# IDEA-Research/MP-Former

Measured on AMD Instinct MI355X. Metric: training images/sec COCO-instance R50 1024x1024, higher is better.
Workload: dtype bf16 (backbone, decoder) + f32 (pixel decoder, losses), as the reference's AMP; 1 GPU; COCO-instance R50, 100 queries, 80 classes, 1024x1024: full train step = R50 backbone + MSDeformAttn pixel decoder (6 layers) + MP masked decoder (9 layers, NUM_DN 1) + Hungarian matching + 60 losses + backward + grad all-reduce + clip + AdamW; head_only_workload=False, global_batch=2, per_gpu_batch=2, parallelism=dp1, msda_offsets=init, full=False, autograd_threads=backward on the launch thread, miopen_find_db=shipped

## Files before the change

include/mpformer_hip.h:

```cpp
#ifndef MPFORMER_HIP_H
#define MPFORMER_HIP_H

#include <stddef.h>
#include <stdint.h>

#ifdef __cplusplus
extern "C" {
#endif

enum { MPF_F32 = 0, MPF_F64 = 1, MPF_BF16 = 2, MPF_U8 = 3, MPF_BITS = 4  };

enum {
    MPF_OK = 0,
    MPF_E_DTYPE = -1,
    MPF_E_SHAPE = -2,
    MPF_E_NULL = -3,
    MPF_E_TOO_LARGE = -4
};

int mpf_abi_version(void);
const char* mpf_last_error(void);


int mpf_msda_forward(const void* value, const int64_t* spatial_shapes,
// ... 315 lines not shown
int mpf_gemm3_nt_h2(const float* a, int64_t lda, const float* a_amax, const float* b, int64_t ldb, const float* b_amax,
                    float* c_part, float* csum_a, float* csum_b, int R, int Mdim, int Ndim, int rows_per_split,
                    int transpose_out, void* stream);
int mpf_gemm3_nt_grouped_h2(const MpfNtItemH2* items, int n_items, int R, int rows_per_split, int64_t split_stride, void* stream);
int mpf_gemm3_conv3x3_h2(const float* x, const float* x_amax, const void* w_planes_h2, const float* w_amax, const float* bias,
                         float* y, float* out_amax, int n_img, int H, int W, int Cin, int Cout, int transposed, void* stream);
int mpf_gemm3_conv3x3_wgrad_h2(const float* dy, const float* dy_amax, const float* x, const float* x_amax, float* c_part,
                               float* csum_dy, int n_img, int H, int W, int Cin, int Cout, int rows_per_split, void* stream);
int mpf_gemm3_tn_h2(const float* a, int64_t lda, const float* a_amax, const void* b_planes_h2, const float* b_amax,
                    const float* bias, const float* c_in, int64_t ldcin, const float* c_in2, int64_t ldcin2,
                    const float* gate, int64_t ldgate, float* c, int64_t ldc, float* out_amax, int M, int N, int K,
                    int relu, void* stream);
int mpf_gemm3_tn_h2_bits(const float* a, int64_t lda, const float* a_amax, const void* b_planes_h2, const float* b_amax,
                         const float* bias, const float* c_in, int64_t ldcin, const float* c_in2, int64_t ldcin2,
                         const unsigned char* gate_bits, int64_t ldgbits, float* c, int64_t ldc, float* out_amax,
                         unsigned char* gate_bits_out, int64_t ldgbits_out, int M, int N, int K, int relu, void* stream);

typedef struct MpfNtItem {
    const float* a;
    int64_t lda;
    const float* b;
    int64_t ldb;
    float* c_part;
    float* csum_a;
    int64_t Mdim, Ndim;
} MpfNtItem;
int mpf_gemm3_nt_grouped(const MpfNtItem* items, int n_items, int R, int rows_per_split, int64_t split_stride, void* stream);

int mpf_gemm3_conv3x3(const float* x, const void* w_planes, const float* bias, float* y, int n_img, int H, int W, int Cin,
                      int Cout, int transposed, void* stream);
int mpf_gemm3_conv3x3_wgrad(const float* dy, const float* x, float* c_part, float* csum_dy, int n_img, int H, int W, int Cin, int Cout,
                            int rows_per_split, void* stream);

int mpf_gemm3_tn_ex(const void* a, int a_dtype, int64_t lda, const void* b_planes, const float* bias, const float* c_in, int64_t ldcin,
                    void* c, int c_dtype, int64_t ldc, int M, int N, int K, int relu, void* stream);
int mpf_gemm3_nt_ex(const void* a, int a_dtype, int64_t lda, const void* b, int b_dtype, int64_t ldb, float* c_part, float* csum_a,
                    int R, int Mdim, int Ndim, int rows_per_split, void* stream);

typedef struct MpfSplitItem {
    const float* src;
    void* dst;
    int64_t rows, cols, transpose, dst_ld, plane_stride, first_block;
} MpfSplitItem;

int mpf_gemm3_split_grouped(const MpfSplitItem* items_device, int n_items, int64_t total_blocks, void* stream);

typedef struct MpfOptItem {
    float* param;
    const float* grad;
    float* exp_avg;
    float* exp_avg_sq;
    int64_t numel, first_block;
    float lr, weight_decay, bc1, bc2_sqrt;
} MpfOptItem;

int mpf_clip_adamw_step(const MpfOptItem* items_device, int n_items, int64_t total_blocks, float max_norm, double beta1,
                        double beta2, double eps, float* partial, float* norm_clip, void* stream);

int mpf_transpose_f32(const float* in, int64_t in_batch_stride, float* out, int64_t out_batch_stride, int B, int R, int C,
                      void* stream);

int mpf_gemm3_nt_reduce(const float* c_part, int64_t c_numel, const float* s_part, int64_t s_numel, int nsplit,
                        float* c_out, float* s_out, void* stream);
int mpf_gemm3_nt_reduce_levels(const float* c_part, int64_t c_numel, const float* s_part, int64_t s_numel, int nsplit,
                               const int64_t* level_of_split, int n_levels, float* c_out, float* lvl_out, float* s_out, void* stream);

// ... 287 lines not shown
```

mp_former_amd/_lib.py:

```python
import ctypes

import torch
import os

_HERE = os.path.dirname(os.path.abspath(__file__))
LIB_PATH = os.path.join(_HERE, "libmpformer_hip.so")
LIB_PATH = os.environ.get("MPF_LIB_PATH", LIB_PATH)
ABI_VERSION = 1

MPF_F32, MPF_F64, MPF_BF16, MPF_U8, MPF_BITS = 0, 1, 2, 3, 4
DTYPE = {torch.float32: MPF_F32, torch.float64: MPF_F64, torch.bfloat16: MPF_BF16, torch.uint8: MPF_U8, torch.bool: MPF_U8}

_lib = None
_status_fns = {}

_c_int = ctypes.c_int
_c_vp = ctypes.c_void_p

SIGNATURES = {
    "mpf_abi_version": (_c_int, []),
    "mpf_last_error": (ctypes.c_char_p, []),
    "mpf_last_kernel": (ctypes.c_char_p, []),
    "mpf_set_option": (_c_int, [ctypes.c_char_p, _c_int]),
    "mpf_match_cost_fused_workspace_bytes": (ctypes.c_size_t, [_c_int] * 5),
# ... 41 lines not shown
    "mpf_attn_forward_kv": (_c_int, [_c_vp, _c_vp, ctypes.c_int64, ctypes.c_int64, _c_vp, _c_vp, _c_int, _c_vp, _c_vp, _c_int, _c_int,
                                     _c_int, _c_int, _c_int, ctypes.c_float, _c_vp, ctypes.c_size_t, _c_vp]),
    "mpf_attn_backward_kv": (_c_int, [_c_vp] * 3 + [ctypes.c_int64] * 2 + [_c_vp] * 5 + [_c_int] + [_c_vp] * 5 + [ctypes.c_int64] * 2
                             + [_c_int] * 6 + [ctypes.c_float, _c_vp, ctypes.c_size_t, _c_vp]),
    "mpf_attn_backward_kv_aux": (_c_int, [_c_vp] * 3 + [ctypes.c_int64] * 2 + [_c_vp] * 5 + [_c_int] + [_c_vp] * 5 + [ctypes.c_int64] * 2
                                 + [_c_int] * 6 + [ctypes.c_float, _c_vp, ctypes.c_size_t, _c_vp, _c_vp]),
    "mpf_attn_bwd_aux_bytes": (ctypes.c_size_t, [_c_int] * 5),
    "mpf_attn_bwd_prep_aux": (_c_int, [_c_vp] * 5 + [_c_int] * 2 + [_c_vp] * 4 + [ctypes.c_size_t] + [_c_int] * 4 + [_c_vp]),
    "mpf_attn_delta": (_c_int, [_c_vp] * 3 + [_c_int] * 3 + [_c_vp]),
    "mpf_attn_bwd_prep": (_c_int, [_c_vp] * 6 + [_c_int] * 4 + [_c_vp]),
    "mpf_win_attn_workspace_bytes": (ctypes.c_size_t, [_c_int] * 5),
    "mpf_win_attn_forward": (_c_int, [_c_vp] * 3 + [_c_int] * 7 + [ctypes.c_float, _c_vp]),
    "mpf_win_attn_backward": (_c_int, [_c_vp] * 6 + [_c_int] * 7 + [ctypes.c_float, _c_vp, ctypes.c_size_t, _c_vp]),
    "mpf_gemm3_split": (_c_int, [_c_vp, _c_int, _c_int, _c_int, _c_vp, _c_vp]),
    "mpf_gemm3_tn": (_c_int, [_c_vp, ctypes.c_int64, _c_vp, _c_int, _c_vp, _c_vp, _c_vp, ctypes.c_int64, _c_vp, ctypes.c_int64,
                           _c_vp, ctypes.c_int64, _c_vp, ctypes.c_int64, _c_int, _c_int, _c_int, _c_int, _c_vp]),
    "mpf_gemm3_nt": (_c_int, [_c_vp, ctypes.c_int64, _c_vp, ctypes.c_int64, _c_vp, ctypes.c_int64, _c_int, _c_vp, _c_vp, _c_vp,
                           _c_int, _c_int, _c_int, _c_int, _c_int, _c_vp]),
    "mpf_amax_f32": (_c_int, [_c_vp, ctypes.c_int64, _c_vp, _c_vp]),
    "mpf_amax_f32_grouped": (_c_int, [_c_vp, _c_int, ctypes.c_int64, _c_vp]),
    "mpf_h2_range_stats": (_c_int, [_c_vp, _c_int, _c_int, ctypes.c_int64, _c_vp, _c_int, _c_vp, _c_vp]),
    "mpf_gemm3_split_grouped_h2": (_c_int, [_c_vp, _c_int, ctypes.c_int64, _c_vp]),
    "mpf_gemm3_tn_h2": (_c_int, [_c_vp, ctypes.c_int64, _c_vp, _c_vp, _c_vp, _c_vp, _c_vp, ctypes.c_int64, _c_vp, ctypes.c_int64,
                              _c_vp, ctypes.c_int64, _c_vp, ctypes.c_int64, _c_vp, _c_int, _c_int, _c_int, _c_int, _c_vp]),
    "mpf_gemm3_tn_h2_bits": (_c_int, [_c_vp, ctypes.c_int64, _c_vp, _c_vp, _c_vp, _c_vp, _c_vp, ctypes.c_int64, _c_vp, ctypes.c_int64,
                                   _c_vp, ctypes.c_int64, _c_vp, ctypes.c_int64, _c_vp, _c_vp, ctypes.c_int64,
                                   _c_int, _c_int, _c_int, _c_int, _c_vp]),
    "mpf_gemm3_nt_h2": (_c_int, [_c_vp, ctypes.c_int64, _c_vp, _c_vp, ctypes.c_int64, _c_vp, _c_vp, _c_vp, _c_vp,
                              _c_int, _c_int, _c_int, _c_int, _c_int, _c_vp]),
    "mpf_gemm3_nt_grouped_h2": (_c_int, [_c_vp, _c_int, _c_int, _c_int, ctypes.c_int64, _c_vp]),
    "mpf_gemm3_conv3x3_h2": (_c_int, [_c_vp] * 7 + [_c_int] * 6 + [_c_vp]),
    "mpf_gemm3_conv3x3_wgrad_h2": (_c_int, [_c_vp, _c_vp, _c_vp, _c_vp, _c_vp, _c_vp, _c_int, _c_int, _c_int, _c_int, _c_int, _c_int, _c_vp]),
    "mpf_gemm3_nt_grouped": (_c_int, [_c_vp, _c_int, _c_int, _c_int, ctypes.c_int64, _c_vp]),
    "mpf_small_gemm_bf16": (_c_int, [_c_vp, ctypes.c_int64, ctypes.c_int64, _c_vp, _c_vp, ctypes.c_int64, ctypes.c_int64, _c_vp, _c_vp,
                                     ctypes.c_int64, _c_vp, ctypes.c_int64, _c_vp, _c_int, _c_int, _c_int, _c_int, _c_vp]),
    "mpf_encoder_fields": (_c_int, []),
    "mpf_encoder_forward": (_c_int, [_c_vp, _c_vp]),
    "mpf_encoder_bwd_fields": (_c_int, []),
    "mpf_encoder_backward": (_c_int, [_c_vp, _c_vp]),
    "mpf_decoder_layer_struct_bytes": (ctypes.c_uint64, [_c_int]),
    "mpf_decoder_layer_scratch_bytes": (ctypes.c_uint64, [_c_int] * 6),
    "mpf_decoder_layer_forward": (_c_int, [_c_vp, _c_vp]),
    "mpf_next_attn_mask_scratch_bytes": (ctypes.c_size_t, [_c_int, _c_int]),
    "mpf_next_attn_mask": (_c_int, [_c_vp, _c_vp]),
    "mpf_lin256_res_ln_forward": (_c_int, [_c_vp] * 11 + [_c_int, ctypes.c_float, _c_vp]),
    "mpf_ln256_mlp3_forward": (_c_int, [_c_vp] * 10 + [_c_int, ctypes.c_float, _c_vp]),
    "mpf_decoder_layer_backward": (_c_int, [_c_vp, _c_vp, _c_vp]),
    "mpf_qpos_operand_forward": (_c_int, [_c_vp, _c_vp, _c_vp, _c_int, _c_int, _c_vp]),
    "mpf_qpos_backward": (_c_int, [_c_vp, _c_vp, _c_vp, _c_vp, _c_int, _c_int, _c_vp]),
    "mpf_decoder_layer_pos_struct_bytes": (ctypes.c_uint64, []),
    "mpf_decoder_layer_pos_scratch_bytes": (ctypes.c_uint64, [_c_int] * 6),
    "mpf_decoder_layer_pos_forward": (_c_int, [_c_vp, _c_vp, _c_vp]),
    "mpf_decoder_layer_pos_backward": (_c_int, [_c_vp, _c_vp, _c_vp, _c_vp]),
    "mpf_pool_features": (_c_int, [_c_vp, _c_int, _c_vp] + [_c_int] * 6 + [_c_vp]),
    "mpf_pool_features_cl": (_c_int, [_c_vp, ctypes.c_int64, _c_int, _c_vp, _c_int, _c_int, _c_int, _c_int, _c_int, _c_int, _c_vp]),
    "mpf_mask_head_bits": (_c_int, [_c_vp, ctypes.c_int64, ctypes.c_int64, _c_vp, _c_vp, _c_int, _c_vp, _c_vp] + [_c_int] * 3 + [_c_vp]),
    "mpf_lsa_assign": (_c_int, [_c_vp, _c_vp, _c_int, _c_int, ctypes.c_int64] + [_c_vp] * 7),
    "mpf_lsa_assign_status": (_c_int, [_c_vp, _c_vp, _c_int, _c_int, ctypes.c_int64] + [_c_vp] * 8),
    "mpf_mask_block_empty": (_c_int, [_c_vp, _c_vp] + [_c_int] * 5 + [_c_vp]),
    "mpf_mp_open_counts": (_c_int, [_c_vp, _c_int, _c_int, _c_vp, _c_vp]),
    "mpf_mp_noise_rows": (_c_int, [_c_vp] * 3 + [_c_int] * 4 + [ctypes.c_double, ctypes.c_uint64, ctypes.c_uint64, _c_vp, _c_vp]),
    "mpf_gemm_nt_bf16_workspace_bytes": (ctypes.c_size_t, [_c_int] * 4),
    "mpf_gemm_nt_bf16": (_c_int, [_c_vp, ctypes.c_int64, _c_vp, ctypes.c_int64, _c_vp, _c_vp, _c_int, _c_int, _c_int, _c_int, _c_vp,
                                  ctypes.c_size_t, _c_vp]),
    "mpf_gemm3_nt_reduce": (_c_int, [_c_vp, ctypes.c_int64, _c_vp, ctypes.c_int64, _c_int, _c_vp, _c_vp, _c_vp]),
    "mpf_grouped_scale_cast": (_c_int, [_c_vp, _c_int, ctypes.c_int64, _c_int, _c_int, _c_vp]),
# ... 256 lines not shown
```

mp_former_amd/backbone.py:

```python
import numpy as np
import torch
import torch.nn.functional as F
from torch import nn

from . import _lib
from ._h2d import upload


class FrozenBatchNorm2d(nn.Module):

    def __init__(self, num_features, eps=1e-5):
        super().__init__()
        self.eps = eps
        self.register_buffer("weight", torch.ones(num_features))
        self.register_buffer("bias", torch.zeros(num_features))
        self.register_buffer("running_mean", torch.zeros(num_features))
        self.register_buffer("running_var", torch.ones(num_features))

    def scale_bias(self):
        b = self._buffers
        w, bb, rm, rv = b["weight"], b["bias"], b["running_mean"], b["running_var"]
        c = self.__dict__.get("_sb_cache")
        if (c is None or c[0] is not w or c[1] is not bb or c[2] is not rm or c[3] is not rv
                or c[4] != (w._version, bb._version, rm._version, rv._version)):
            with torch.no_grad():
                scale = w * (rv + self.eps).rsqrt()
                c = (w, bb, rm, rv, (w._version, bb._version, rm._version, rv._version), scale,
                     (bb - rm * scale).float().contiguous())
            self.__dict__["_sb_cache"] = c
        return c[5], c[6]

    def forward(self, x):
# ... 82 lines not shown

    @staticmethod
    def forward(ctx, x):
        N, C, H, W = x.shape
        OH, OW = (H - 1) // 2 + 1, (W - 1) // 2 + 1
        y = torch.empty((N, C, OH, OW), dtype=x.dtype, device=x.device, memory_format=torch.channels_last)
        code = torch.empty((N, OH, OW, C), dtype=torch.uint8, device=x.device)
        _lib.call("mpf_maxpool3x3s2_forward", x.device, x.data_ptr(), y.data_ptr(), code.data_ptr(), N, H, W, C,
                  _lib.stream_ptr(x.device))
        ctx.save_for_backward(code)
        ctx.in_shape = (N, C, H, W)
        return y

    @staticmethod
    def backward(ctx, gy):
        (code,) = ctx.saved_tensors
        N, C, H, W = ctx.in_shape
        if gy.dtype != torch.bfloat16 or not gy.is_contiguous(memory_format=torch.channels_last):
            gy = gy.to(torch.bfloat16).contiguous(memory_format=torch.channels_last)
        gx = torch.empty((N, C, H, W), dtype=gy.dtype, device=gy.device, memory_format=torch.channels_last)
        _lib.call("mpf_maxpool3x3s2_backward", gy.device, gy.data_ptr(), code.data_ptr(), gx.data_ptr(), N, H, W, C,
                  _lib.stream_ptr(gy.device))
        return gx


def max_pool_3x3_s2(x):
    if (x.is_cuda and x.dim() == 4 and x.dtype == torch.bfloat16 and x.shape[1] % 8 == 0 and 256 % (x.shape[1] // 8) == 0
            and x.is_contiguous(memory_format=torch.channels_last)):
        return _MaxPool3x3s2.apply(x)
    return F.max_pool2d(x, kernel_size=3, stride=2, padding=1)


def conv_bn(conv, bn, x, folded=None, res=None, relu=True, fork=False):
    if folded is not None:
        w, shift = folded
    else:
        scale, shift = bn.scale_bias()
        w = conv.weight * scale.view(-1, 1, 1, 1)
    y = F.conv2d(x, w, None, conv.stride, conv.padding, conv.dilation, conv.groups)
    return bias_act_fork(y, shift, res) if fork else bias_act(y, shift, res, relu)


def _dense(t):
    return t.is_contiguous() or (t.dim() == 4 and t.is_contiguous(memory_format=torch.channels_last))


_gsc_layouts = {}


def _grouped_scale_cast(srcs, scales, out_dtype):
    dev = srcs[0].device
    key = tuple([(t.shape, t.stride()) for t in srcs] + [id(sc) for sc in scales] + [out_dtype])
    lay = _gsc_layouts.get(key)
    if lay is None:
        numels = [t.numel() for t in srcs]
        offs, tot, blk = [], 0, 0
        table = np.zeros((len(srcs), 6), dtype=np.int64)
        for i, (t, sc) in enumerate(zip(srcs, scales)):
            assert _dense(t) and sc.dtype == torch.float32 and sc.is_contiguous() and sc.numel() == t.shape[0]
            offs.append(tot)
            table[i, 2:] = (sc.data_ptr(), numels[i], numels[i] // t.shape[0], blk)
            tot += (numels[i] + 63) & ~63
            blk += (numels[i] + 2047) // 2048
        esz = torch.empty(0, dtype=out_dtype).element_size()
        lay = (table, np.asarray(offs, dtype=np.int64) * esz, tot, blk, [(o, n, t.shape, t.stride()) for o, n, t in zip(offs, numels, srcs)],
               list(scales))
        if len(_gsc_layouts) > 64:
            _gsc_layouts.clear()
        _gsc_layouts[key] = lay
    table, offs_b, tot, blk, views, _ = lay
    out = torch.empty(tot, dtype=out_dtype, device=dev)
    table[:, 0] = [t.data_ptr() for t in srcs]
    table[:, 1] = offs_b + out.data_ptr()
    items = upload(table.reshape(-1), dev)
    _lib.call("mpf_grouped_scale_cast", dev, items.data_ptr(), len(srcs), blk, _lib.DTYPE[srcs[0].dtype], _lib.DTYPE[out_dtype],
              _lib.stream_ptr(dev))
    return [out[o:o + n].as_strided(shp, std) for o, n, shp, std in views]


class _FoldCast(torch.autograd.Function):

    @staticmethod
    def forward(ctx, dtype, scales, *weights):
        ctx.scales = scales
        ws = [p.detach() for p in weights]
        native = (ws[0].is_cuda and all(w.dtype == torch.float32 and _dense(w) for w in ws)
                  and dtype in (None, torch.float32, torch.bfloat16))
        ctx.native = native
        if native:
            return tuple(_grouped_scale_cast(ws, scales, dtype or torch.float32))
        w = torch._foreach_mul(ws, [s_.view(-1, 1, 1, 1) for s_ in scales])
        if dtype is None:
            return tuple(w)
        outs = [torch.empty_like(t, dtype=dtype) for t in w]
        torch._foreach_copy_(outs, w)
        return tuple(outs)

    @staticmethod
    def backward(ctx, *grads):
        if ctx.native and all(g is not None and g.dtype == grads[0].dtype for g in grads) \
                and grads[0].dtype in (torch.float32, torch.bfloat16):
            gs = [g if _dense(g) else g.contiguous() for g in grads]
            return (None, None, *_grouped_scale_cast(gs, ctx.scales, torch.float32))
        g32 = [torch.empty_like(g, dtype=torch.float32) for g in grads]
        torch._foreach_copy_(g32, list(grads))
        torch._foreach_mul_(g32, [s_.view(-1, 1, 1, 1) for s_ in ctx.scales])
        return (None, None, *g32)


_PAIR_NAMES = (("conv1", "norm1"), ("conv2", "norm2"), ("conv3", "norm3"), ("shortcut", "shortcut_norm"))


class Bottleneck(nn.Module):
    def __init__(self, cin, cmid, cout, stride):
        super().__init__()
        self.shortcut = None
        if cin != cout or stride != 1:
            self.shortcut = nn.Conv2d(cin, cout, 1, stride=stride, bias=False)
            self.shortcut_norm = FrozenBatchNorm2d(cout)
        self.conv1 = nn.Conv2d(cin, cmid, 1, bias=False)
        self.norm1 = FrozenBatchNorm2d(cmid)
        self.conv2 = nn.Conv2d(cmid, cmid, 3, stride=stride, padding=1, bias=False)
        self.norm2 = FrozenBatchNorm2d(cmid)
        self.conv3 = nn.Conv2d(cmid, cout, 1, bias=False)
        self.norm3 = FrozenBatchNorm2d(cout)

    def pairs(self):
        m = self._modules
        p = self.__dict__.get("_pairs")
        if p is not None:
            names = _PAIR_NAMES if len(p) == 4 else _PAIR_NAMES[:3]
            if (m.get("shortcut") is None) != (len(p) == 3) or any(c is not m.get(cn) or n is not m.get(nn_) for (c, n), (cn, nn_) in zip(p, names)):
                p = None
        if p is None:
            p = [(self.conv1, self.norm1), (self.conv2, self.norm2), (self.conv3, self.norm3)]
            if self.shortcut is not None:
                p.append((self.shortcut, self.shortcut_norm))
            self.__dict__["_pairs"] = p
        return p

# ... 3 lines not shown
    def forward_fork(self, xs, fw=None):
        f = fw if fw is not None else [None] * 4
        x_main, x_skip = xs
        p = self.pairs()
        out = conv_bn(p[0][0], p[0][1], x_main, f[0])
        out = conv_bn(p[1][0], p[1][1], out, f[1])
        sc = x_skip if len(p) == 3 else conv_bn(p[3][0], p[3][1], x_skip, f[3], relu=False)
        return conv_bn(p[2][0], p[2][1], out, f[2], res=sc, fork=True)


class ResNet50(nn.Module):
    def __init__(self):
        super().__init__()
        self.stem_conv = nn.Conv2d(3, 64, 7, stride=2, padding=3, bias=False)
        self.stem_norm = FrozenBatchNorm2d(64)
        cfg = [("res2", 3, 64, 256, 1), ("res3", 4, 128, 512, 2), ("res4", 6, 256, 1024, 2), ("res5", 3, 512, 2048, 2)]
        cin = 64
        self.stage_names = []
        for name, n, cmid, cout, stride in cfg:
            blocks = []
            for i in range(n):
                blocks.append(Bottleneck(cin, cmid, cout, stride if i == 0 else 1))
                cin = cout
            setattr(self, name, nn.Sequential(*blocks))
            self.stage_names.append(name)
        for m in self.modules():
            if isinstance(m, nn.Conv2d):
                nn.init.kaiming_normal_(m.weight, mode="fan_out", nonlinearity="relu")

    @staticmethod
    def _fold_group(pairs, dtype):
        sb = [bn.scale_bias() for _, bn in pairs]
        scales = [s_ for s_, _ in sb]
        ws = _FoldCast.apply(dtype, scales, *[c.weight for c, _ in pairs])
        return [(w, b_) for w, (_, b_) in zip(ws, sb)]

    def forward(self, x):
        return self.forward_stages(x, self.stage_names, stem=True)

    def forward_stages(self, x, names, stem=False):
        return run_stages(x, [(n, getattr(self, n)) for n in names], (self.stem_conv, self.stem_norm) if stem else None)


def run_stages(x, stages, stem=None):
    dtype = torch.get_autocast_dtype("cuda") if (torch.is_autocast_enabled() and x.is_cuda) else None
    if stem is not None:
        st = ResNet50._fold_group([stem], dtype)
        x = conv_bn(stem[0], stem[1], x, st[0])
        x = max_pool_3x3_s2(x)
    out = {}
    for name, stage in stages:
        blocks = list(stage)
        folded = ResNet50._fold_group([p for b in blocks for p in b.pairs()], dtype)
        k = 0
        xs = x if isinstance(x, tuple) else (x, x)
        for b in blocks:
            n = len(b.pairs())
            xs = b.forward_fork(xs, folded[k:k + n])
            k += n
        x = xs
        out[name] = xs[0]
    return out
```

mp_former_amd/csrc/gemm3.hip:

```cpp
#include <hip/hip_runtime.h>

#include <algorithm>
#include <atomic>
#include <stdint.h>
#include <stdio.h>

#include "mpf_common.h"
#include "amax.h"
#ifndef G3_PRIO
#define G3_PRIO 1
#endif

namespace {

typedef __attribute__((ext_vector_type(8))) __bf16 bf16x8;
typedef __attribute__((ext_vector_type(4))) float f32x4;

constexpr int kBM = 128;
constexpr int kBK = 32;
constexpr int kThreads = 256;
constexpr int kAKc = kBM * 16;

struct G3 {
    const float* a;
// ... 941 lines not shown
        g3_tn_tile<64, A2>(p, lds, (p.tm0 + tm) * kBM, tn * 64);
    }
}

struct G3N {
    const float* a;
    const float* b;
    const float* b2;
    float* c;
    float* csum_a;
    float* csum_b;
    int64_t lda, ldb, ldb2;
    int R, Mdim, Ndim, b2_rows, rows_per_split, nsplit, tiles_m, tiles_n, ntiles, transpose_out;
    unsigned a_bytes, b_bytes;
    int cv_H, cv_W, cv_cin;
    int64_t c_ss, csa_ss, csb_ss;
    const float* a_amax;
    const float* b_amax;
};
constexpr int kNtGroupMax = 8;
struct G3NG {
    G3N it[kNtGroupMax];
    int tile_end[kNtGroupMax];
    int n_items, ntiles;
};

template <int BN, bool BF, bool CV, bool A16, bool B16, bool H2 = false>
__device__ __forceinline__ void gemm3_nt_tile(const G3N& p, const int tile)
{
    static_assert(!((A16 || B16) && (BF || CV || BN != 128)), "mixed-precision operands: plain 128-column tiles only");
    static_assert(!(H2 && (BF || A16 || B16)), "fp16 x 2 form: fp32 operands only");
    constexpr int NJ = BN / 32;
    constexpr int kBKc = BN * 16;
    constexpr int kPl = H2 ? 2 : 3;
    constexpr int kAbytes = kPl * 4 * kAKc;
    constexpr int kBunits = 4 * BN;
    __shared__ __attribute__((aligned(16))) unsigned char lds[kAbytes + kPl * 4 * kBKc];
    float sc_a = 1.f, sc_b = 1.f, inv_a = 1.f, inv_b = 1.f;
    if constexpr (H2) {
        h2_scale(amax_read(p.a_amax), &sc_a, &inv_a);
        h2_scale(amax_read(p.b_amax), &sc_b, &inv_b);
    }
    (void)sc_a; (void)sc_b;

    const int tn = tile % p.tiles_n, tm = (tile / p.tiles_n) % p.tiles_m, sp = tile / (p.tiles_n * p.tiles_m);
    const int m0 = tm * kBM, n0 = tn * BN;
    const int r_begin = sp * p.rows_per_split, r_end = min(p.R, r_begin + p.rows_per_split);

    const int tid = threadIdx.x, lane = tid & 63, wave = tid >> 6;
    const int wr = wave >> 1, wc = wave & 1;


    const int am = tid & 127, akc = __builtin_amdgcn_readfirstlane(tid >> 7);
    const bool a_col_ok = m0 + am < p.Mdim;
    const int acolx = min(m0 + am, p.Mdim - 1);
    int bn_[2], bkc_[2], bcolx[2];
    bool b_ok[2], b_col_ok[2];
    int b2row[2];
#pragma unroll
    for (int i = 0; i < 2; ++i) {
        const int u = tid + i * kThreads;
        b_ok[i] = u < kBunits;
        bn_[i] = u % BN;
        bkc_[i] = min(u / BN, 3);
        if (BN == 128) bkc_[i] = __builtin_amdgcn_readfirstlane(bkc_[i]);
        b_col_ok[i] = b_ok[i] && n0 + bn_[i] < p.Ndim;
        bcolx[i] = min(n0 + bn_[i], p.Ndim - 1);
// ... 1095 lines not shown
        if (l < L) {
            *reinterpret_cast<float2*>(lvl_out + (int64_t)l * sn + j) = acc[l];
            tot.x += acc[l].x; tot.y += acc[l].y;
        }
    *reinterpret_cast<float2*>(s_out + j) = tot;
}

extern "C" int mpf_gemm3_nt_reduce_levels(const float* c_part, int64_t c_numel, const float* s_part, int64_t s_numel, int nsplit,
                                          const int64_t* level_of_split, int n_levels, float* c_out, float* lvl_out, float* s_out,
                                          void* stream)
{
    if (!c_part || !c_out || !s_part || !s_out || !lvl_out || !level_of_split) return mpf::fail(MPF_E_NULL, "gemm3_nt_reduce_levels: NULL buffer");
    if (nsplit <= 0 || c_numel <= 0 || s_numel <= 0 || c_numel % 4 || s_numel % 4 || n_levels < 1 || n_levels > 4)
        return mpf::fail(MPF_E_SHAPE, "gemm3_nt_reduce_levels: sizes must be positive multiples of 4, 1..4 levels");
    const int64_t quads = (c_numel + s_numel) / 2;
    mpf::set_kernel("nt_reduce_levels_kernel");
    hipLaunchKernelGGL(nt_reduce_levels_kernel, dim3((unsigned)((quads + 255) / 256)), dim3(256), 0, (hipStream_t)stream, c_part, c_numel,
                       s_part, s_numel, nsplit, level_of_split, n_levels, c_out, lvl_out, s_out);
    return mpf::check(hipGetLastError(), "mpf_gemm3_nt_reduce_levels");
}

extern "C" int mpf_gemm3_nt_reduce(const float* c_part, int64_t c_numel, const float* s_part, int64_t s_numel, int nsplit,
                                   float* c_out, float* s_out, void* stream)
{
    if (!c_part || !c_out || (s_numel > 0 && (!s_part || !s_out))) return mpf::fail(MPF_E_NULL, "gemm3_nt_reduce: NULL buffer");
    if (nsplit <= 0 || c_numel <= 0 || s_numel < 0 || c_numel % 4 || s_numel % 4)
        return mpf::fail(MPF_E_SHAPE, "gemm3_nt_reduce: sizes must be positive multiples of 4");
    const int64_t quads = (c_numel + s_numel) / 2;
    mpf::set_kernel("nt_reduce_kernel");
    hipLaunchKernelGGL(nt_reduce_kernel<true>, dim3((unsigned)((quads + 255) / 256)), dim3(256), 0, (hipStream_t)stream, c_part,
                       c_numel, s_part, s_numel, nsplit, c_out, s_out);
    return mpf::check(hipGetLastError(), "mpf_gemm3_nt_reduce");
}
```

Baseline: 86.36 images/sec.

## Defer backbone conv weight-grads and compute them in one grouped bf16 GEMM launch

Backbone 1x1 and stride-1 3x3 convs now skip the weight-gradient part of MIOpen's convolution_backward and only record (dy, x). At the fold-cast backward, all recorded weight gradients for the group are computed together by a new grouped bf16 NT GEMM kernel with split-K partials. A second kernel reduces the partials, applies the BN scale and writes fp32 gradients. This is meant to replace many separate MIOpen wgrad calls with a couple of launches, at the cost of keeping activations and gradients alive longer and a bf16-rounding step that may differ slightly from the reference. It also shrinks LDS use in the bf16 tile path (kPl = 1 when BF).

```diff
diff --git a/include/mpformer_hip.h b/include/mpformer_hip.h
--- a/include/mpformer_hip.h
+++ b/include/mpformer_hip.h
@@ -371,6 +371,28 @@
 int mpf_gemm3_conv3x3_wgrad(const float* dy, const float* x, float* c_part, float* csum_dy, int n_img, int H, int W, int Cin, int Cout,
                             int rows_per_split, void* stream);
 
+#define MPF_CONV_WGRAD_GROUP_MAX 12
+#define MPF_CONV_WGRAD_1X1 0
+#define MPF_CONV_WGRAD_3X3 1
+typedef struct MpfConvWgradItem {
+    const void* dy;
+    int64_t ld_dy;
+    const void* x;
+    int64_t ld_x;
+    const float* scale;
+    float* out;
+    int64_t out_stride_co, out_stride_ci, out_stride_tap;
+    int64_t ws_offset;
+    int R, Cout, Cin, kind, H, W, rows_per_split, reserved;
+} MpfConvWgradItem;
+typedef struct MpfConvWgradPlan {
+    int64_t ws_offset, ws_bytes;
+    int rows_per_split, nsplit, tiles, launch;
+} MpfConvWgradPlan;
+int mpf_conv_wgrad_group_max(void);
+int mpf_conv_wgrad_plan(const MpfConvWgradItem* items, int n_items, int slots, MpfConvWgradPlan* plans, size_t* workspace_bytes);
+int mpf_conv_wgrad_bf16_grouped(const MpfConvWgradItem* items, int n_items, void* workspace, size_t workspace_bytes, void* stream);
+
 int mpf_gemm3_tn_ex(const void* a, int a_dtype, int64_t lda, const void* b_planes, const float* bias, const float* c_in, int64_t ldcin,
                     void* c, int c_dtype, int64_t ldc, int M, int N, int K, int relu, void* stream);
 int mpf_gemm3_nt_ex(const void* a, int a_dtype, int64_t lda, const void* b, int b_dtype, int64_t ldb, float* c_part, float* csum_a,
diff --git a/mp_former_amd/_lib.py b/mp_former_amd/_lib.py
--- a/mp_former_amd/_lib.py
+++ b/mp_former_amd/_lib.py
@@ -97,6 +97,9 @@
     "mpf_gemm3_conv3x3_h2": (_c_int, [_c_vp] * 7 + [_c_int] * 6 + [_c_vp]),
     "mpf_gemm3_conv3x3_wgrad_h2": (_c_int, [_c_vp, _c_vp, _c_vp, _c_vp, _c_vp, _c_vp, _c_int, _c_int, _c_int, _c_int, _c_int, _c_int, _c_vp]),
     "mpf_gemm3_nt_grouped": (_c_int, [_c_vp, _c_int, _c_int, _c_int, ctypes.c_int64, _c_vp]),
+    "mpf_conv_wgrad_group_max": (_c_int, []),
+    "mpf_conv_wgrad_plan": (_c_int, [_c_vp, _c_int, _c_int, _c_vp, ctypes.POINTER(ctypes.c_size_t)]),
+    "mpf_conv_wgrad_bf16_grouped": (_c_int, [_c_vp, _c_int, _c_vp, ctypes.c_size_t, _c_vp]),
     "mpf_small_gemm_bf16": (_c_int, [_c_vp, ctypes.c_int64, ctypes.c_int64, _c_vp, _c_vp, ctypes.c_int64, ctypes.c_int64, _c_vp, _c_vp,
                                      ctypes.c_int64, _c_vp, ctypes.c_int64, _c_vp, _c_int, _c_int, _c_int, _c_int, _c_vp]),
     "mpf_encoder_fields": (_c_int, []),
diff --git a/mp_former_amd/backbone.py b/mp_former_amd/backbone.py
--- a/mp_former_amd/backbone.py
+++ b/mp_former_amd/backbone.py
@@ -1,3 +1,6 @@
+import ctypes
+import os
+
 import numpy as np
 import torch
 import torch.nn.functional as F
@@ -146,12 +149,18 @@
 
 
 def conv_bn(conv, bn, x, folded=None, res=None, relu=True, fork=False):
+    y = None
     if folded is not None:
-        w, shift = folded
+        w, shift = folded[0], folded[1]
+        if len(folded) == 4:
+            kind = _wgrad_kind(conv, x, w)
+            if kind is not None:
+                y = _ConvDeferredWgrad.apply(x, w, folded[2], folded[3], kind)
     else:
         scale, shift = bn.scale_bias()
         w = conv.weight * scale.view(-1, 1, 1, 1)
-    y = F.conv2d(x, w, None, conv.stride, conv.padding, conv.dilation, conv.groups)
+    if y is None:
+        y = F.conv2d(x, w, None, conv.stride, conv.padding, conv.dilation, conv.groups)
     return bias_act_fork(y, shift, res) if fork else bias_act(y, shift, res, relu)
 
 
@@ -192,10 +201,146 @@
     return [out[o:o + n].as_strided(shp, std) for o, n, shp, std in views]
 
 
+_WGRAD_ROUTES = ("native", "miopen")
+_wgrad_route = os.environ.get("MPF_BACKBONE_WGRAD", "native")
+if _wgrad_route not in _WGRAD_ROUTES:
+    raise ValueError(f"MPF_BACKBONE_WGRAD={_wgrad_route!r}: expected one of {_WGRAD_ROUTES}")
+_CW_1X1, _CW_3X3 = 0, 1
+
+
+def set_wgrad_route(route):
+    global _wgrad_route
+    if route not in _WGRAD_ROUTES:
+        raise ValueError(f"wgrad route {route!r}: expected one of {_WGRAD_ROUTES}")
+    prev, _wgrad_route = _wgrad_route, route
+    return prev
+
+
+class _WgradRecord:
+    __slots__ = ("items",)
+
+    def __init__(self):
+        self.items = {}
+
+
+def _wgrad_kind(conv, x, w):
+    if not (torch.is_grad_enabled() and w.requires_grad and x.is_cuda and x.dtype == torch.bfloat16 and w.dtype == torch.bfloat16
+            and x.dim() == 4 and x.is_contiguous(memory_format=torch.channels_last)):
+        return None
+    if conv.stride != (1, 1) or conv.dilation != (1, 1) or conv.groups != 1 or x.shape[1] % 4 != 0:
+        return None
+    if conv.kernel_size == (1, 1) and conv.padding == (0, 0):
+        return _CW_1X1
+    if conv.kernel_size == (3, 3) and conv.padding == (1, 1) and x.shape[1] % 128 == 0 and x.shape[3] % 8 == 0:
+        return _CW_3X3
+    return None
+
+
+_placeholders = {}
+
+
+def _placeholder(w):
+    key = (w.device, w.dtype)
+    z = _placeholders.get(key)
+    if z is None:
+        z = _placeholders[key] = torch.zeros((), dtype=w.dtype, device=w.device)
+    return z.expand(w.shape)
+
+
+class _ConvDeferredWgrad(torch.autograd.Function):
+
+    @staticmethod
+    def forward(ctx, x, w, rec, idx, kind):
+        ctx.save_for_backward(x, w)
+        ctx.rec, ctx.idx, ctx.kind = rec, idx, kind
+        return F.conv2d(x, w, None, 1, 1 if kind == _CW_3X3 else 0)
+
+    @staticmethod
+    def backward(ctx, gy):
+        x, w = ctx.saved_tensors
+        need_x, need_w = ctx.needs_input_grad[0], ctx.needs_input_grad[1]
+        deferred = need_w and gy.dtype == torch.bfloat16 and gy.is_contiguous(memory_format=torch.channels_last)
+        gx = gw = None
+        if need_x or (need_w and not deferred):
+            pad = [1, 1] if ctx.kind == _CW_3X3 else [0, 0]
+            gx, gw, _ = torch.ops.aten.convolution_backward(gy, x, w, None, [1, 1], pad, [1, 1], False, [0, 0], 1,
+                                                            [need_x, need_w and not deferred, False])
+        if deferred:
+            ctx.rec.items[ctx.idx] = (gy, x, ctx.kind)
+            gw = _placeholder(w)
+        return gx, gw, None, None, None
+
+
+class _CwItem(ctypes.Structure):
+    _fields_ = [("dy", ctypes.c_void_p), ("ld_dy", ctypes.c_int64), ("x", ctypes.c_void_p), ("ld_x", ctypes.c_int64),
+                ("scale", ctypes.c_void_p), ("out", ctypes.c_void_p), ("out_stride_co", ctypes.c_int64),
+                ("out_stride_ci", ctypes.c_int64), ("out_stride_tap", ctypes.c_int64), ("ws_offset", ctypes.c_int64),
+                ("R", ctypes.c_int), ("Cout", ctypes.c_int), ("Cin", ctypes.c_int), ("kind", ctypes.c_int), ("H", ctypes.c_int),
+                ("W", ctypes.c_int), ("rows_per_split", ctypes.c_int), ("reserved", ctypes.c_int)]
+
+
+class _CwPlan(ctypes.Structure):
+    _fields_ = [("ws_offset", ctypes.c_int64), ("ws_bytes", ctypes.c_int64), ("rows_per_split", ctypes.c_int),
+                ("nsplit", ctypes.c_int), ("tiles", ctypes.c_int), ("launch", ctypes.c_int)]
+
+
+def conv_wgrad_plan(items, slots=0, device=torch.device("cpu")):
+    n = len(items)
+    plans = (_CwPlan * n)()
+    ws = ctypes.c_size_t(0)
+    _lib.call("mpf_conv_wgrad_plan", device, items, n, slots, plans, ctypes.byref(ws))
+    for it, pl in zip(items, plans):
+        it.rows_per_split, it.ws_offset = pl.rows_per_split, pl.ws_offset
+    return list(plans), ws.value
+
+
+def conv_wgrad_item(R, Cout, Cin, kind, H=0, W=0, out_strides=None):
+    taps = 9 if kind == _CW_3X3 else 1
+    sco, sci, stap = out_strides if out_strides is not None else (taps * Cin, 1, Cin)
+    return _CwItem(None, Cout, None, Cin, None, None, sco, sci, stap, 0, R, Cout, Cin, kind, H, W, 0, 0)
+
+
+_cw_layouts = {}
+
+
+def _conv_wgrad_grouped(entries, scales):
+    dev = entries[0][0].device
+    key = (dev, _lib.option_generation()) + tuple((gy.shape, x.shape[1], kind) for gy, x, kind in entries)
+    lay = _cw_layouts.get(key)
+    if lay is None:
+        arr = (_CwItem * len(entries))()
+        views, tot = [], 0
+        for i, (gy, x, kind) in enumerate(entries):
+            N, Cout, H, W = gy.shape
+            Cin = x.shape[1]
+            arr[i] = conv_wgrad_item(N * H * W, Cout, Cin, kind, H, W)
+            shape = (Cout, Cin, 3, 3) if kind == _CW_3X3 else (Cout, Cin, 1, 1)
+            stride = (9 * Cin, 1, 3 * Cin, Cin) if kind == _CW_3X3 else (Cin, 1, 1, 1)
+            views.append((tot, Cout * Cin * shape[2] * shape[3], shape, stride))
+            tot += (views[-1][1] + 63) & ~63
+        _, ws_bytes = conv_wgrad_plan(arr, 0, dev)
+        if len(_cw_layouts) > 64:
+            _cw_layouts.clear()
+        lay = _cw_layouts[key] = (arr, ws_bytes, views, tot)
+    arr, ws_bytes, views, tot = lay
+    stream = _lib.stream_ptr(dev)
+    out = torch.empty(tot, dtype=torch.float32, device=dev)
+    ws = _lib.scratch("conv_wgrad", dev, stream, ws_bytes)
+    base = out.data_ptr()
+    for it, (gy, x, _), sc, (off, _, _, _) in zip(arr, entries, scales, views):
+        assert sc.dtype == torch.float32 and sc.is_contiguous() and sc.numel() == it.Cout
+        it.dy, it.x, it.scale, it.out = gy.data_ptr(), x.data_ptr(), sc.data_ptr(), base + 4 * off
+    _lib.call("mpf_conv_wgrad_bf16_grouped", dev, arr, len(entries), ws.data_ptr(), ws.numel(), stream)
+    return [out[o:o + n].as_strided(shp, std) for o, n, shp, std in views]
+
+
 class _FoldCast(torch.autograd.Function):
 
     @staticmethod
     def forward(ctx, dtype, scales, *weights):
+        ctx.rec = None
+        if weights and isinstance(weights[0], _WgradRecord):
+            ctx.rec, weights = weights[0], weights[1:]
         ctx.scales = scales
         ws = [p.detach() for p in weights]
         native = (ws[0].is_cuda and all(w.dtype == torch.float32 and _dense(w) for w in ws)
@@ -212,14 +357,32 @@
 
     @staticmethod
     def backward(ctx, *grads):
-        if ctx.native and all(g is not None and g.dtype == grads[0].dtype for g in grads) \
+        rec = ctx.rec
+        if rec is None:
+            return (None, None, *_FoldCast._cast_back(ctx.native, grads, ctx.scales))
+        deferred, rec.items = rec.items, {}
+        if not deferred:
+            return (None, None, None, *_FoldCast._cast_back(ctx.native, grads, ctx.scales))
+        out = [None] * len(grads)
+        idx = list(deferred)
+        for i, g in zip(idx, _conv_wgrad_grouped([deferred[i] for i in idx], [ctx.scales[i] for i in idx])):
+            out[i] = g
+        rest = [i for i in range(len(grads)) if i not in deferred]
+        if rest:
+            for i, g in zip(rest, _FoldCast._cast_back(ctx.native, [grads[i] for i in rest], [ctx.scales[i] for i in rest])):
+                out[i] = g
+        return (None, None, None, *out)
+
+    @staticmethod
+    def _cast_back(native, grads, scales):
+        if native and all(g is not None and g.dtype == grads[0].dtype for g in grads) \
                 and grads[0].dtype in (torch.float32, torch.bfloat16):
             gs = [g if _dense(g) else g.contiguous() for g in grads]
-            return (None, None, *_grouped_scale_cast(gs, ctx.scales, torch.float32))
+            return _grouped_scale_cast(gs, scales, torch.float32)
         g32 = [torch.empty_like(g, dtype=torch.float32) for g in grads]
         torch._foreach_copy_(g32, list(grads))
-        torch._foreach_mul_(g32, [s_.view(-1, 1, 1, 1) for s_ in ctx.scales])
-        return (None, None, *g32)
+        torch._foreach_mul_(g32, [s_.view(-1, 1, 1, 1) for s_ in scales])
+        return g32
 
 
 _PAIR_NAMES = (("conv1", "norm1"), ("conv2", "norm2"), ("conv3", "norm3"), ("shortcut", "shortcut_norm"))
@@ -289,7 +452,12 @@
     def _fold_group(pairs, dtype):
         sb = [bn.scale_bias() for _, bn in pairs]
         scales = [s_ for s_, _ in sb]
-        ws = _FoldCast.apply(dtype, scales, *[c.weight for c, _ in pairs])
+        weights = [c.weight for c, _ in pairs]
+        if _wgrad_route == "native" and dtype == torch.bfloat16 and torch.is_grad_enabled():
+            rec = _WgradRecord()
+            ws = _FoldCast.apply(dtype, scales, rec, *weights)
+            return [(w, b_, rec, i) for i, (w, (_, b_)) in enumerate(zip(ws, sb))]
+        ws = _FoldCast.apply(dtype, scales, *weights)
         return [(w, b_) for w, (_, b_) in zip(ws, sb)]
 
     def forward(self, x):
diff --git a/mp_former_amd/csrc/gemm3.hip b/mp_former_amd/csrc/gemm3.hip
--- a/mp_former_amd/csrc/gemm3.hip
+++ b/mp_former_amd/csrc/gemm3.hip
@@ -997,7 +997,7 @@
     static_assert(!(H2 && (BF || A16 || B16)), "fp16 x 2 form: fp32 operands only");
     constexpr int NJ = BN / 32;
     constexpr int kBKc = BN * 16;
-    constexpr int kPl = H2 ? 2 : 3;
+    constexpr int kPl = BF ? 1 : H2 ? 2 : 3;
     constexpr int kAbytes = kPl * 4 * kAKc;
     constexpr int kBunits = 4 * BN;
     __shared__ __attribute__((aligned(16))) unsigned char lds[kAbytes + kPl * 4 * kBKc];
@@ -2159,3 +2159,5 @@
                        c_numel, s_part, s_numel, nsplit, c_out, s_out);
     return mpf::check(hipGetLastError(), "mpf_gemm3_nt_reduce");
 }
+
+#include "gemm3_conv_wgrad.h"
diff --git a/mp_former_amd/csrc/gemm3_conv_wgrad.h b/mp_former_amd/csrc/gemm3_conv_wgrad.h
--- /dev/null
+++ b/mp_former_amd/csrc/gemm3_conv_wgrad.h
@@ -0,0 +1,232 @@
+
+namespace {
+
+constexpr int kCwMax = MPF_CONV_WGRAD_GROUP_MAX;
+
+struct G3NC {
+    G3N it[kCwMax];
+    int tile_end[kCwMax];
+    unsigned char cv[kCwMax];
+    int n_items, ntiles;
+};
+static_assert(sizeof(G3NC) <= 4096, "kernel arguments are limited to 4 KB");
+
+__global__ __launch_bounds__(kThreads, 2) void gemm3_nt_conv_group_kernel(G3NC g)
+{
+    const int per_xcd = (g.ntiles + 7) >> 3;
+    const int tile = ((int)blockIdx.x & 7) * per_xcd + ((int)blockIdx.x >> 3);
+    if (tile >= g.ntiles) return;
+    int i = 0;
+    while (i + 1 < g.n_items && tile >= g.tile_end[i]) ++i;
+    const int first = i ? g.tile_end[i - 1] : 0;
+    if (g.cv[i]) gemm3_nt_tile<128, true, true, false, false>(g.it[i], tile - first);
+    else gemm3_nt_tile<128, true, false, false, false>(g.it[i], tile - first);
+}
+
+struct CwRed {
+    const float* part;
+    const float* scale;
+    float* out;
+    int64_t sco, sci, stap;
+    int nsplit, Cout, K, Cin, vec;
+};
+struct CwRedGroup {
+    CwRed it[kCwMax];
+    int block_end[kCwMax];
+    int n_items;
+};
+static_assert(sizeof(CwRedGroup) <= 4096, "kernel arguments are limited to 4 KB");
+
+__global__ __launch_bounds__(256) void conv_wgrad_reduce_kernel(CwRedGroup g)
+{
+    int i = 0;
+    while (i + 1 < g.n_items && (int)blockIdx.x >= g.block_end[i]) ++i;
+    const CwRed& p = g.it[i];
+    const int first = i ? g.block_end[i - 1] : 0;
+    const int64_t total = (int64_t)p.Cout * p.K;
+    const int64_t e = ((int64_t)((int)blockIdx.x - first) * 256 + threadIdx.x) * 4;
+    if (e >= total) return;
+    const float* src = p.part + e;
+    float4 acc = make_float4(0.f, 0.f, 0.f, 0.f);
+    int sp = 0;
+    for (; sp + 4 <= p.nsplit; sp += 4) {
+        float4 t[4];
+#pragma unroll
+        for (int k = 0; k < 4; ++k) t[k] = *reinterpret_cast<const float4*>(src + (int64_t)(sp + k) * total);
+#pragma unroll
+        for (int k = 0; k < 4; ++k) { acc.x += t[k].x; acc.y += t[k].y; acc.z += t[k].z; acc.w += t[k].w; }
+    }
+    for (; sp < p.nsplit; ++sp) {
+        const float4 t = *reinterpret_cast<const float4*>(src + (int64_t)sp * total);
+        acc.x += t.x; acc.y += t.y; acc.z += t.z; acc.w += t.w;
+    }
+    auto bf16_rn = [](float f) -> float {
+        unsigned u = __float_as_uint(f);
+        u += 0x7fffu + ((u >> 16) & 1u);
+        return __uint_as_float(u & 0xffff0000u);
+    };
+    const int co = (int)(e / p.K), k = (int)(e - (int64_t)co * p.K);
+    const int tap = k / p.Cin, ci = k - tap * p.Cin;
+    const float s = p.scale[co];
+    const float4 o = make_float4(bf16_rn(acc.x) * s, bf16_rn(acc.y) * s, bf16_rn(acc.z) * s, bf16_rn(acc.w) * s);
+    float* dst = p.out + (int64_t)co * p.sco + (int64_t)tap * p.stap + (int64_t)ci * p.sci;
+    if (p.vec) {
+        *reinterpret_cast<float4*>(dst) = o;
+    } else {
+        dst[0] = o.x; dst[p.sci] = o.y; dst[2 * p.sci] = o.z; dst[3 * p.sci] = o.w;
+    }
+}
+
+inline int cw_taps(const MpfConvWgradItem& it) { return it.kind == MPF_CONV_WGRAD_3X3 ? 9 : 1; }
+
+int cw_check_item(const MpfConvWgradItem& it)
+{
+    if (it.kind != MPF_CONV_WGRAD_1X1 && it.kind != MPF_CONV_WGRAD_3X3) return mpf::fail(MPF_E_SHAPE, "conv_wgrad: kind is MPF_CONV_WGRAD_1X1 or _3X3");
+    if (it.R <= 0 || it.Cout <= 0 || it.Cin <= 0 || it.Cin % 4 != 0 || it.Cout > (1 << 20) || it.Cin > (1 << 20))
+        return mpf::fail(MPF_E_SHAPE, "conv_wgrad: sizes must be positive, Cin a multiple of 4");
+    if ((int64_t)it.Cout * cw_taps(it) * it.Cin >= (1ll << 30)) return mpf::fail(MPF_E_TOO_LARGE, "conv_wgrad: a gradient of 2^30 elements or more");
+    if (it.ld_dy < it.Cout || it.ld_x < it.Cin) return mpf::fail(MPF_E_SHAPE, "conv_wgrad: a row stride is shorter than the row");
+    if (it.kind == MPF_CONV_WGRAD_3X3) {
+        if (it.H <= 0 || it.W <= 0 || it.W % 8 != 0 || it.Cin % 128 != 0 || it.R % (it.H * it.W) != 0)
+            return mpf::fail(MPF_E_SHAPE, "conv_wgrad: a 3x3 item needs W % 8 == 0, Cin % 128 == 0 and R = images * H * W");
+    }
+    return 0;
+}
+
+inline int cw_launches(int n_items) { return cdiv(n_items, kCwMax); }
+inline int cw_launch_begin(int n_items, int launch)
+{
+    const int per = cdiv(n_items, cw_launches(n_items));
+    return std::min(n_items, launch * per);
+}
+
+void cw_plan_launch(const MpfConvWgradItem* items, int n, int slots, MpfConvWgradPlan* plans)
+{
+    int tiles[kCwMax], steps[kCwMax], cap[kCwMax], max_steps = 1;
+    for (int i = 0; i < n; ++i) {
+        const MpfConvWgradItem& it = items[i];
+        const int64_t K = (int64_t)cw_taps(it) * it.Cin;
+        tiles[i] = cdiv(it.Cout, kBM) * cdiv((int)K, 128);
+        steps[i] = cdiv(it.R, kBK);
+        const int64_t operand = 2 * (int64_t)it.R * (it.Cout + K), part = 4 * (int64_t)it.Cout * K;
+        cap[i] = (int)std::max<int64_t>(1, std::min<int64_t>(operand / part, steps[i]));
+        max_steps = std::max(max_steps, steps[i]);
+    }
+    int best_L = max_steps;
+    double best_cost = 0.0;
+    for (int L = max_steps; L >= 1; --L) {
+        int64_t wgs = 0;
+        int longest = 0;
+        for (int i = 0; i < n; ++i) {
+            const int ns = std::min(cap[i], cdiv(steps[i], L));
+            wgs += (int64_t)tiles[i] * cdiv(steps[i], cdiv(steps[i], ns));
+            longest = std::max(longest, cdiv(steps[i], ns));
+        }
+        if (wgs > 3 * (int64_t)slots && L < max_steps) break;
+        const double cost = (double)cdiv((int)wgs, slots) * (longest + 8);
+        if (L == max_steps || cost < best_cost) { best_cost = cost; best_L = L; }
+    }
+    for (int i = 0; i < n; ++i) {
+        const int ns = std::min(cap[i], cdiv(steps[i], best_L));
+        const int len = cdiv(steps[i], ns);
+        plans[i].rows_per_split = len * kBK;
+        plans[i].nsplit = cdiv(steps[i], len);
+        plans[i].tiles = tiles[i] * plans[i].nsplit;
+    }
+}
+
+}
+
+extern "C" int mpf_conv_wgrad_group_max(void) { return kCwMax; }
+
+extern "C" int mpf_conv_wgrad_plan(const MpfConvWgradItem* items, int n_items, int slots, MpfConvWgradPlan* plans,
+                                   size_t* workspace_bytes)
+{
+    if (!items || !plans || !workspace_bytes) return mpf::fail(MPF_E_NULL, "conv_wgrad_plan: NULL argument");
+    if (n_items <= 0 || slots < 0) return mpf::fail(MPF_E_SHAPE, "conv_wgrad_plan: n_items must be positive, slots >= 0 (0: the current device's)");
+    for (int i = 0; i < n_items; ++i)
+        if (int rc = cw_check_item(items[i])) return rc;
+    if (slots == 0) slots = g3_slots();
+    size_t off = 0;
+    for (int l = 0; l < cw_launches(n_items); ++l) {
+        const int b = cw_launch_begin(n_items, l), e = cw_launch_begin(n_items, l + 1);
+        cw_plan_launch(items + b, e - b, slots, plans + b);
+        for (int i = b; i < e; ++i) {
+            plans[i].launch = l;
+            plans[i].ws_offset = (int64_t)off;
+            plans[i].ws_bytes = (int64_t)mpf::align256((size_t)plans[i].nsplit * items[i].Cout * cw_taps(items[i]) * items[i].Cin * sizeof(float));
+            off += (size_t)plans[i].ws_bytes;
+        }
+    }
+    *workspace_bytes = off;
+    return 0;
+}
+
+extern "C" int mpf_conv_wgrad_bf16_grouped(const MpfConvWgradItem* items, int n_items, void* workspace, size_t workspace_bytes,
+                                           void* stream)
+{
+    hipStream_t st = (hipStream_t)stream;
+    if (!items || !workspace) return mpf::fail(MPF_E_NULL, "conv_wgrad_bf16_grouped: NULL argument");
+    if (n_items <= 0) return mpf::fail(MPF_E_SHAPE, "conv_wgrad_bf16_grouped: n_items must be positive");
+    for (int i = 0; i < n_items; ++i) {
+        const MpfConvWgradItem& it = items[i];
+        if (!it.dy || !it.x || !it.scale || !it.out) return mpf::fail(MPF_E_NULL, "conv_wgrad_bf16_grouped: NULL buffer in an item");
+        if (int rc = cw_check_item(it)) return rc;
+        if (it.rows_per_split <= 0 || it.rows_per_split % kBK != 0)
+            return mpf::fail(MPF_E_SHAPE, "conv_wgrad_bf16_grouped: rows_per_split must be a positive multiple of 32");
+        const size_t need = (size_t)cdiv(it.R, it.rows_per_split) * it.Cout * cw_taps(it) * it.Cin * sizeof(float);
+        if (it.ws_offset < 0 || it.ws_offset % 16 != 0 || (size_t)it.ws_offset + need > workspace_bytes)
+            return mpf::fail(MPF_E_SHAPE, "conv_wgrad_bf16_grouped: an item's partial sums do not fit its slice of the workspace");
+        for (int j = 0; j < i; ++j) {
+            const MpfConvWgradItem& o = items[j];
+            const size_t need_o = (size_t)cdiv(o.R, o.rows_per_split) * o.Cout * cw_taps(o) * o.Cin * sizeof(float);
+            if ((size_t)it.ws_offset < (size_t)o.ws_offset + need_o && (size_t)o.ws_offset < (size_t)it.ws_offset + need)
+                return mpf::fail(MPF_E_SHAPE, "conv_wgrad_bf16_grouped: two items share workspace");
+        }
+    }
+    for (int l = 0; l < cw_launches(n_items); ++l) {
+        const int b = cw_launch_begin(n_items, l), e = cw_launch_begin(n_items, l + 1);
+        G3NC g{};
+        CwRedGroup r{};
+        Work w{0.0, 0.0};
+        double red_bytes = 0.0;
+        int blocks = 0;
+        for (int i = b; i < e; ++i) {
+            const MpfConvWgradItem& it = items[i];
+            const bool cv = it.kind == MPF_CONV_WGRAD_3X3;
+            G3N& p = g.it[i - b];
+            float* part = reinterpret_cast<float*>(static_cast<unsigned char*>(workspace) + it.ws_offset);
+            if (int rc = g3n_fill(p, "conv_wgrad_bf16_grouped", it.dy, it.ld_dy, 2, it.x, it.ld_x, 2, part, nullptr, it.R, it.Cout, it.Cin,
+                                  it.rows_per_split))
+                return rc;
+            if (cv) {
+                p.Ndim = 9 * it.Cin; p.c_ss = (int64_t)p.Mdim * p.Ndim; p.csb_ss = p.Ndim;
+                p.cv_H = it.H; p.cv_W = it.W; p.cv_cin = it.Cin;
+            }
+            g3n_tiles(p, kBM, 128);
+            g.cv[i - b] = cv ? 1 : 0;
+            g.ntiles += p.ntiles;
+            g.tile_end[i - b] = g.ntiles;
+            const Work wi = g3n_work(p, 2.0, 2.0);
+            w.bytes += wi.bytes; w.flops += wi.flops;
+
+            CwRed& q = r.it[i - b];
+            q.part = part; q.scale = it.scale; q.out = it.out;
+            q.sco = it.out_stride_co; q.sci = it.out_stride_ci; q.stap = it.out_stride_tap;
+            q.nsplit = p.nsplit; q.Cout = it.Cout; q.K = p.Ndim; q.Cin = it.Cin;
+            q.vec = q.sci == 1 && q.sco % 4 == 0 && (!cv || q.stap % 4 == 0) && ((uintptr_t)it.out & 15) == 0;
+            blocks += cdiv(it.Cout * p.Ndim, 1024);
+            r.block_end[i - b] = blocks;
+            red_bytes += 4.0 * (p.nsplit + 1) * it.Cout * p.Ndim;
+        }
+        g.n_items = r.n_items = e - b;
+        if (int rc = g3_launch(g3n_route((const void*)gemm3_nt_conv_group_kernel, "gemm3_nt_group_kernel<bf16 conv>",
+                                         "mpf_conv_wgrad_bf16_grouped", g.ntiles), g, st, w))
+            return rc;
+        Route rr;
+        rr.fn = (const void*)conv_wgrad_reduce_kernel; rr.name = "conv_wgrad_reduce_kernel"; rr.what = "mpf_conv_wgrad_bf16_grouped(reduce)";
+        rr.blocks = blocks;
+        if (int rc = g3_launch(rr, r, st, Work{red_bytes, 0.0})) return rc;
+    }
+    return 0;
+}
```

Result: faster. 88.06 images/sec, median of 6 (+2.0%).
